# Alisah-Ozcan/GPU-NTT

Measured on AMD Instinct MI355X. Metric: forward-NTTs/sec + achieved HBM GB/s, 64-bit Merge N=2^16 batch=1024, higher is better.
Workload: dtype u64; 1 GPU; Merge-NTT Data64 log2N=16 batch=1024 forward (BASELINE configs[1]); log2N=16, batch_per_gpu=1024, reduction_poly=X_N_minus, modulus=576460756061519873, in_place=True, api=dropin, parallelism=batch-shard x1

## Files before the change

### gpu-ntt_amd/__init__.py

```python
import ctypes
import os
import subprocess
from dataclasses import dataclass
from typing import Optional

import numpy as np

_HERE = os.path.dirname(os.path.abspath(__file__))
LIB_PATH = os.environ.get("GPUNTT_LIB") or os.path.join(_HERE, "lib", "libgpuntt.so")
CSRC = os.path.join(_HERE, "csrc")

FORWARD, INVERSE = 0, 1
PerPolynomial, PerCoefficient = 0, 1
X_N_plus, X_N_minus = 0, 1

GPUNTT_OK = 0
_ERR_INVALID, _ERR_HIP = -1, -2


class GpuNttError(RuntimeError):
    """HipException / CudaException of the C++ API (failed launch)."""


class _M32(ctypes.Structure):
# ... 52 lines not shown
              "innerprod_plan_owns_workspace", "innerprod_plan_destroy", "innerprod_constants",
              "innerprod_reference",
              "keyswitch_plan_workspace_bytes", "keyswitch_plan_scratch_bytes", "keyswitch_plan_create",
              "keyswitch_plan_mod_up", "keyswitch_plan_mod_down", "keyswitch_plan_decompose",
              "keyswitch_plan_switch_digits", "keyswitch_plan_apply", "keyswitch_plan_hoisted_scratch_bytes",
              "keyswitch_plan_rotate_hoisted", "keyswitch_plan_hoisted_sum_scratch_bytes",
              "keyswitch_plan_rotate_hoisted_sum", "keyswitch_plan_multiply_relinearize",
              "keyswitch_plan_multiply_relinearize_sum", "keyswitch_plan_owns_workspace",
              "keyswitch_plan_destroy", "keyswitch_constants", "keyswitch_reference_mod_up",
              "keyswitch_reference_mod_down",
              "keyswitch_plan_workspace_bytes_rescale", "keyswitch_plan_create_rescale",
              "keyswitch_plan_rescale_limbs", "keyswitch_plan_rescale_scratch_bytes",
              "keyswitch_plan_mod_down_rescale", "keyswitch_plan_rescale",
              "keyswitch_plan_multiply_relinearize_rescale", "keyswitch_plan_multiply_relinearize_sum_rescale",
              "keyswitch_plan_rotate_hoisted_sum_rescale", "keyswitch_reference_mod_down_rescale",
              "keyswitch_reference_rescale")
    for s in ("u32", "u64")] + ["gpuntt_release_workspaces", "gpuntt_set_option", "gpuntt_galois_element_u32",
                                "gpuntt_automorphism_index_map"]

ENV_OPTIONS = {"GPUNTT_PATH": ("path", None), "GPUNTT_U32_E32": ("u32_e32", lambda v: int(v, 0)),
               "GPUNTT_TWO_SWEEP_BIG": ("two_sweep_big", None)}


TEST_HOOKS = {"no_scratch", "rns_force_fallback", "u32_e32", "reset_predictions", "two_sweep_big", "baseconv_ksplit",
              "keyswitch_split", "keyswitch_hoist_chunk", "contig_p4"}
TEST_PATHS = {"fast-strict", "generic-capped"}


def set_option(name, value):
    name, value = str(name), str(value)
    if name in TEST_HOOKS or (name == "path" and value in TEST_PATHS):
        return set_test_hook(name, value)
    _check(load_library().gpuntt_set_option(name.encode(), value.encode()))


def set_test_hook(name, value):
    _check(load_library().gpuntt_test_set_hook(str(name).encode(), str(value).encode()))


def contig_p4_launches():
    fn = load_library().gpuntt_test_contig_p4_launches
    fn.restype = ctypes.c_ulonglong
    return int(fn())


def alloc_count():
    fn = load_library().gpuntt_test_alloc_count
    fn.restype = ctypes.c_ulonglong
    return int(fn())


def scratch_stats():
    out = (ctypes.c_ulonglong * 6)()
    _check(load_library().gpuntt_test_scratch_stats(out))
    names = ("graph_owned", "died", "pooled", "reused", "chains_erased", "chains")
    return dict(zip(names, (int(v) for v in out)))


class launch_log:

    def __enter__(self):
        _check(load_library().gpuntt_test_launch_log_start())
        self.kernels = []
        return self

    def __exit__(self, *exc):
# ... 1144 lines not shown
```

### gpu-ntt_amd/csrc/c_api.cpp

```cpp
#include <algorithm>
#include <cstring>
#include <exception>
#include <initializer_list>
#include <stdexcept>
#include <string>
#include <vector>

#include "gpuntt/ntt_4step/ntt_4step.cuh"
#include "gpuntt/ntt_merge/galois.cuh"
#include "gpuntt/ntt_merge/ntt.cuh"
#include "gpuntt/rns/base_conversion.cuh"
#include "gpuntt/rns/inner_product.cuh"
#include "gpuntt/rns/key_switch.cuh"
#include "gpuntt_c.h"
#include "hoisted_rotation_internal.hpp"
#include "test_hooks.h"

namespace gpuntt
{
    namespace host
    {
        template <typename T> void debug_recip_norm(const T* q, T* out, unsigned long long count, hipStream_t stream);
        bool set_test_hook(const char* name, const char* value);
        void launch_log_start();
        size_t launch_log_take(std::string& out, size_t capacity);
        unsigned long long alloc_count();
        void scratch_stats(unsigned long long out[6]);
        unsigned long long contig_p4_launches();
    }
}

using namespace gpuntt;

namespace
{
    thread_local std::string g_last_error;

    template <typename F> int guarded(F&& f)
    {
        try
        {
            f();
            return GPUNTT_OK;
        }
        catch (const std::invalid_argument& e)
        {
            g_last_error = e.what();
            return GPUNTT_ERR_INVALID_ARGUMENT;
        }
        catch (const HipException& e)
        {
            g_last_error = e.what();
            return GPUNTT_ERR_HIP;
        }
        catch (const std::exception& e)
        {
            g_last_error = e.what();
            return GPUNTT_ERR_UNKNOWN;
        }
    }

// ... 420 lines not shown
    }
    int gpuntt_version(void) { return 101; }

    int gpuntt_test_set_hook(const char* name, const char* value)
    {
        return guarded([&] {
            if (!host::set_test_hook(name, value))
                throw std::invalid_argument("Unknown option or value!");
        });
    }
    int gpuntt_test_launch_log_start(void)
    {
        return guarded([] { host::launch_log_start(); });
    }
    int gpuntt_test_launch_log_take(char* buf, int capacity)
    {
        std::string s;
        const size_t room = (buf != nullptr && capacity > 0) ? static_cast<size_t>(capacity - 1) : 0;
        const size_t need = host::launch_log_take(s, room);
        if (buf != nullptr && capacity > 0)
        {
            std::memcpy(buf, s.data(), s.size());
            buf[s.size()] = '\0';
        }
        return static_cast<int>(need) + 1;
    }
    unsigned long long gpuntt_test_alloc_count(void) { return host::alloc_count(); }

    int gpuntt_test_scratch_stats(unsigned long long out[6])
    {
        return guarded([&] { host::scratch_stats(out); });
    }
    unsigned long long gpuntt_test_contig_p4_launches(void) { return host::contig_p4_launches(); }
    int gpuntt_test_keyswitch_hoist_chunk(int word_bytes, int digits, int n_power)
    {
        if ((word_bytes != 4 && word_bytes != 8) || digits < 1 || digits > INNERPROD_MAX_DIGITS || n_power < 1 ||
            n_power > 28)
            return -1;
        return host::hoist_chunk_log(static_cast<size_t>(word_bytes), digits, n_power, host::HOIST_LOG_MAX);
    }
    int gpuntt_test_keyswitch_hoist_sum_chunk(int word_bytes, int digits, int n_power)
    {
        if ((word_bytes != 4 && word_bytes != 8) || digits < 1 || digits > INNERPROD_MAX_DIGITS || n_power < 1 ||
            n_power > 28)
            return -1;
        return host::hoist_chunk_log(static_cast<size_t>(word_bytes), digits, n_power, host::HOIST_SUM_LOG_MAX);
    }

    int gpuntt_galois_element_u32(int steps, int n_power, int conjugation, uint32_t* elt_host)
    {
        GPUNTT_NEED(elt_host)
        return guarded([&] {
            *elt_host = conjugation ? GaloisElementForConjugation(n_power) : GaloisElementForRotation(steps, n_power);
        });
    }
    int gpuntt_automorphism_index_map(int n_power, uint32_t galois_elt, int reduction_poly, int domain,
                                      uint32_t* map_host)
    {
        GPUNTT_NEED(map_host)
        return guarded([&] {
            if (n_power <= 0 || n_power >= 29)
                throw std::invalid_argument("Invalid n_power range!");
            if (reduction_poly != GPUNTT_X_N_PLUS && reduction_poly != GPUNTT_X_N_MINUS)
                throw std::invalid_argument("Invalid reduction_poly!");
            if (domain != GPUNTT_DOMAIN_NTT && domain != GPUNTT_DOMAIN_COEFFICIENT)
                throw std::invalid_argument("Invalid domain!");
// ... 701 lines not shown
```

### gpu-ntt_amd/csrc/contig_p4_map.hpp

```cpp
#pragma once

#if defined(__HIPCC__) || defined(__CUDACC__)
#define GPUNTT_P4_HD __host__ __device__
#else
#define GPUNTT_P4_HD
#endif

namespace gpuntt
{
    namespace kern
    {
        namespace p4
        {
            constexpr int TLOG = 12;
            constexpr int K = 10;
            constexpr int RB = 4;
            constexpr int NT = 256;
            constexpr int POLYS = 1 << (TLOG - K);
            constexpr int ROUNDS = 3;
            constexpr int LDS_ELEMS = (1 << TLOG) + (1 << (TLOG - 4)) + 16 * (POLYS - 1);

            GPUNTT_P4_HD constexpr int window(int r) { return r == 0 ? 6 : (r == 1 ? 4 : 0); }

            GPUNTT_P4_HD constexpr unsigned thread_of(int r, unsigned t)
            {
                return r == 0 ? t : ((t & 15u) | ((t >> 6) << 4) | (((t >> 4) & 3u) << 6));
            }
            GPUNTT_P4_HD constexpr unsigned elem(int r, unsigned t, unsigned j)
            {
                const unsigned u = thread_of(r, t);
                const int w = window(r);
                return (u & ((1u << w) - 1u)) | (j << w) | ((u >> w) << (w + RB));
            }
            GPUNTT_P4_HD constexpr unsigned elem_out(unsigned t, unsigned j)
            {
                return (t & 63u) | ((j & 3u) << 6) | ((t >> 6) << 8) | ((j >> 2) << K);
            }
            GPUNTT_P4_HD constexpr unsigned lds_slot(unsigned e) { return e + (e >> 4) + ((e >> K) << 4); }
            GPUNTT_P4_HD constexpr unsigned long long mem_offset(unsigned e, unsigned long long poly_stride)
            {
                return static_cast<unsigned long long>(e >> K) * poly_stride + (e & ((1u << K) - 1u));
            }
            GPUNTT_P4_HD constexpr unsigned ring_pos(unsigned seg, unsigned e) { return (seg << K) | (e & ((1u << K) - 1u)); }

            GPUNTT_P4_HD constexpr unsigned tw_uniform_index(int n, unsigned seg, unsigned blk, int p, unsigned kk)
            {
                return (1u << (n - 1 - p)) + (((seg << K) | (blk << 8)) >> (p + 1)) + kk;
            }
            GPUNTT_P4_HD constexpr unsigned tw_lane_index(int n, unsigned seg, unsigned t, int p, unsigned kk)
            {
                const unsigned group = ((seg & 3u) << 6) | ((t >> 6) << 4) | (t & 15u);
                return (1u << (n - 1 - p)) + (seg >> 2) * ((8u >> p) * NT) + kk * NT + group;
            }
        }
    }
}
```

### gpu-ntt_amd/csrc/lazy_launch.hpp

```cpp
#pragma once

#include <hip/hip_runtime.h>

#include <string>

#include "launch.hpp"
#include "merge_lazy_kernels.hpp"

namespace gpuntt
{
    namespace host
    {
        constexpr int LAZY_MAX_N_POWER = 28;

        constexpr int lazy_u32_tile_override() { return 0; }
        constexpr int lazy_u64_big_tiles() { return 14; }

        bool lazy_two_sweep_big();
        bool lazy_contig_p4();
        void note_contig_p4_launch();
        unsigned long long contig_p4_launches();
        constexpr int LAZY_P4_N_POWER = 16;
        constexpr unsigned long long lazy_u32_small_batch() { return 0x7fffffffull; }
        template <typename T> inline int lazy_tile_log(int n, bool inverse = false, unsigned long long polys = 0)
        {
            if (sizeof(T) == 8)
            {
                const int big = lazy_u64_big_tiles();
                if (n == 13 && big >= 13)
                    return 13;
                if (n == 14 && big >= 14 && !inverse && polys >= 256)
                    return 14;
                if (n == 21 && big >= 13)
                    return 13;
                if (n == 22 && big >= 14)
                    return 14;
                if ((n == 23 || n == 24) && !inverse && lazy_two_sweep_big())
                    return 14;
                return 12;
            }
            if (n <= 12)
                return 12;
            {
                const unsigned long long small = lazy_u32_small_batch();
                if (n == 13 && small != 0 && (polys == 0 ? small >= 0x7fffffffull : polys <= small))
                    return 13;
            }
            if (n <= 14)
                return 14;
            const int forced = lazy_u32_tile_override();
            if (forced != 0)
                return forced;
            return (n >= 20 && n <= 22) ? 14 : 12;
        }

// ... 504 lines not shown
```

### gpu-ntt_amd/csrc/lazy_launch_impl.hpp

```cpp
#pragma once

#include "lazy_launch.hpp"

namespace gpuntt
{
    namespace host
    {
        template <typename T, int TLOG, bool INV, bool CONTIG, int K, int IN_BOUND, bool LAST, int LIMSEL = 0, bool P4 = false,
                  int CAP = 0>
        inline void launch_lazy_one(const kern::LazyArgsT<T>& a, unsigned grid, hipStream_t stream)
        {
            if constexpr (P4)
                note_contig_p4_launch();
            GPUNTT_LAUNCH_FAMILY(LIMSEL, (kern::merge_pass_lazy<T, TLOG, INV, CONTIG, K, IN_BOUND, LAST, LIMSEL, 0, P4, CAP>), dim3(grid),
                               dim3(kern::LTile<TLOG>::NT), 0, stream, a);
            GPUNTT_HIP_CHECK(hipGetLastError());
        }

        template <typename T, int TLOG, bool INV, int LIMSEL = 0>
        void dispatch_tl(const Pass& p, bool in_first, bool last, const kern::LazyArgsT<T>& a,
                         hipStream_t stream)
        {
            constexpr int LIM = lazy::Mod<T, LIMSEL>::LIMIT;
            constexpr int TILE = kern::LTile<TLOG>::TILE;
            const unsigned long long tiles = (a.total + TILE - 1) >> TLOG;
            if (tiles == 0)
                return;
            if (tiles > 0x7fffffffull)
                throw std::invalid_argument("batch_size * N too large for one launch");
            const unsigned grid = lazy_grid_cap<T, LIMSEL>(tiles, a.go_flag);
            constexpr bool CAPPED = sizeof(T) == 8 && !INV && TLOG == 12 && (LIM == 16 || LIM == 31);
            constexpr int CAP10 = CAPPED ? FwdBounds<CAPPED ? LIM : 16>::CAP10 : LIM;
            if (!CAPPED && p.cap != 0)
                throw std::invalid_argument("internal: no capped hand-off in this kernel family");
#define GPUNTT_ONE(CONTIG_, K_, IN_, LAST_)                                                      \
    return launch_lazy_one<T, TLOG, INV, CONTIG_, K_, IN_, LAST_, LIMSEL>(a, grid, stream)
            if constexpr (sizeof(T) == 8 && TLOG >= 13)
            {
                if (p.contig && p.k == TLOG)
                {
                    if (in_first && last)
                        GPUNTT_ONE(true, TLOG, 1, true);
                    if constexpr (!INV)
                    {
                        if (!in_first && last)
                            GPUNTT_ONE(true, TLOG, LIM, true);
// ... 33 lines not shown
                            case 8: GPUNTT_ONE(true, 8, 1, true);
                            case 9: GPUNTT_ONE(true, 9, 1, true);
                            case 10: GPUNTT_ONE(true, 10, 1, true);
                            case 11: GPUNTT_ONE(true, 11, 1, true);
                            case 12: GPUNTT_ONE(true, 12, 1, true);
                            default: break;
                        }
                    else if constexpr (TLOG == 13)
                    {
                        if (p.k == 13)
                            GPUNTT_ONE(true, 13, 1, true);
                    }
                    else
                        switch (p.k)
                        {
                            case 13: GPUNTT_ONE(true, 13, 1, true);
                            case 14: GPUNTT_ONE(true, 14, 1, true);
                            default: break;
                        }
                }
                else if (!INV && !in_first && last)
                {
                    if constexpr (!INV)
                    {
                        if constexpr (TLOG == 12)
                            switch (p.k)
                            {
                                case 8: GPUNTT_ONE(true, 8, LIM, true);
                                case 9: GPUNTT_ONE(true, 9, LIM, true);
                                case 10:
                                    if constexpr (sizeof(T) == 8)
                                        if (p.p4)
                                        {
                                            if constexpr (CAPPED)
                                                if (fwd_inst_bound(p, TLOG, in_first, last, LIM) == CAP10)
                                                    return launch_lazy_one<T, TLOG, INV, true, 10, CAP10, true, LIMSEL, true>(a, grid, stream);
                                            return launch_lazy_one<T, TLOG, INV, true, 10, LIM, true, LIMSEL, true>(a, grid, stream);
                                        }
                                    if constexpr (CAPPED)
                                        if (fwd_inst_bound(p, TLOG, in_first, last, LIM) == CAP10)
                                            GPUNTT_ONE(true, 10, CAP10, true);
                                    GPUNTT_ONE(true, 10, LIM, true);
                                case 11: GPUNTT_ONE(true, 11, LIM, true);
                                case 12: GPUNTT_ONE(true, 12, LIM, true);
                                default: break;
                            }
                        else if constexpr (TLOG == 14)
                        {
                            if (p.k == 14)
                                GPUNTT_ONE(true, 14, LIM, true);
                            if (p.k == 13)
                                GPUNTT_ONE(true, 13, LIM, true);
                        }
                    }
                }
                else if (INV && in_first && !last)
                {
                    if constexpr (INV)
                    {
                        if constexpr (TLOG == 12)
                            switch (p.k)
                            {
                                case 8: GPUNTT_ONE(true, 8, 1, false);
                                case 9: GPUNTT_ONE(true, 9, 1, false);
                                case 10: GPUNTT_ONE(true, 10, 1, false);
                                case 11: GPUNTT_ONE(true, 11, 1, false);
                                case 12: GPUNTT_ONE(true, 12, 1, false);
                                default: break;
                            }
                        else if constexpr (TLOG == 14)
// ... 371 lines not shown
```

### gpu-ntt_amd/csrc/merge_lazy_kernels.hpp

```cpp
#pragma once

#include "contig_p4_map.hpp"
#include "lazy.hpp"
#include "merge_kernels.hpp"

namespace gpuntt
{
    namespace kern
    {
        template <typename T> struct LazyArgsT
        {
            const void* in;
            T* out;
            const lazy::Tw<T>* tw;
            const Modulus<T>* mods;
            T q;
            T q_bit;
            T q_mu;
            const lazy::Tw<T>* ninv_arr;
            lazy::Tw<T> ninv;
            lazy::NormConst norm;
            const lazy::NormConst* norm_arr;
            const unsigned* go_flag;
            const int* mod_order;
            const int* poly_order;
            const T* mul_in;
            const T* fs_n1;
            const T* fs_n2;
            const T* fs_w;
            int lim;
            int host_allow_31q;
            int n2_log;
            int row_log;
            int batch;
            int col_log;
            int mod_shift;
            unsigned long long total;
            int n;
            int poly_shift;
            int mod_count;
            int p_lo;
            unsigned flags;
        };
        using LazyArgs = LazyArgsT<uint64_t>;

        template <int WL> constexpr int lds_joff(int j)
        {
            return (j << WL) + ((WL >= 4) ? (j << (WL >= 4 ? WL - 4 : 0)) : (j >> (WL < 4 ? 4 - WL : 0)));
        }

        template <int TLOG> struct LTile
        {
            static constexpr int TL = TLOG;
            static constexpr int NT = 1 << (TLOG - R);
            static constexpr int TILE = 1 << TLOG;
            static constexpr int LDS_ELEMS = TILE + (TILE >> 4);
            static constexpr int LDS_ELEMS_FST = TILE + (TILE >> 4) + (TILE >> 5);
        };
        template <int TLOG, bool CONTIG, int K> struct LGeo
        {
            static constexpr int L = CONTIG ? 0 : (TLOG - K);
            static constexpr int NR = (K + R - 1) / R;
        };
        template <int TLOG, bool CONTIG, int K, bool SEG = false> struct LTileMap
        {
            unsigned long long base;
            int p_lo;
            __device__ __forceinline__ explicit LTileMap(unsigned long long flat_base, int row_shift = 0)
                : base(flat_base), p_lo(row_shift)
            {
            }
            __device__ __forceinline__ LTileMap(int n, int pass_p_lo, unsigned long long blk)
            {
                constexpr int L = LGeo<TLOG, CONTIG, K>::L;
                if constexpr (CONTIG)
// ... 123 lines not shown
                                b[j1] = TB;
                            }
                        }
                        g++;
                    }
                    int mx = 0;
                    for (int j = 0; j < EPT; j++)
                    {
                        d.bout[r][j] = b[j];
                        mx = b[j] > mx ? b[j] : mx;
                    }
                    bound_in = mx;
                }
                d.final_bound = (EST && (!whole.ok || whole.out != bound_in)) ? LIMIT + 1 : bound_in;
                return d;
            }
            static constexpr Data d = make();
            static_assert(d.final_bound <= LIMIT, "lazy bound exceeds the headroom");
            static_assert(d.final_bound <= HANDOFF_CAP, "the pass hands over more than its successor was compiled for");
            static_assert(!INV || d.final_bound <= LIMIT / 2, "an inverse pass must hand over values below LIMIT / 2");
        };

        template <typename T, bool INV, bool VQ, bool PLAIN> constexpr bool plans_whole_pass(int limit)
        {
            return !INV && sizeof(T) == 8 && !VQ && PLAIN && (limit == 16 || limit == 31);
        }

        template <int TLOG, typename T = uint32_t> struct LOcc
        {
            static constexpr int WAVES = (TLOG >= 14 && sizeof(T) == 4) ? 8 : 4;
        };

        constexpr int TW_PER_ROUND = EPT - 1;

        template <bool NT_, typename T> __device__ __forceinline__ T ld_stream(const T* p)
        {
            if constexpr (NT_)
                return __builtin_nontemporal_load(p);
            else
                return *p;
        }
        template <bool NT_, typename T> __device__ __forceinline__ void st_stream(T* p, T v)
        {
            if constexpr (NT_)
                __builtin_nontemporal_store(v, p);
            else
                *p = v;
        }

        __device__ __forceinline__ void wave_sync()
        {
            __builtin_amdgcn_fence(__ATOMIC_RELEASE, "wavefront");
            __builtin_amdgcn_wave_barrier();
            __builtin_amdgcn_fence(__ATOMIC_ACQUIRE, "wavefront");
        }

        constexpr int XP_L1 = 5;
        template <int K> __device__ __forceinline__ unsigned xp_swap_fwd(unsigned f)
        {
            constexpr unsigned M = (1u << K) - 1u;
            const unsigned w = f & M;
            return (f & ~M) | ((w & 31u) << (K - XP_L1)) | (w >> XP_L1);
        }
        template <int K> __device__ __forceinline__ unsigned xp_swap_inv(unsigned e)
        {
            return xp_swap_fwd<K>(e);
// ... 24 lines not shown
                else
                    asm volatile("" : "+v"(v[j])::"memory");
            }
        }

        enum class Fst : int
        {
            none = 0,
            nat_rows = 2,
            inv_first = 3
        };
        enum class Xp : int
        {
            none = 0,
            small_fwd = 1,
            small_inv = 2,
            small_nat_fwd = 3,
            small_nat_inv = 4,
            first_gather = 5
        };

        template <typename T, int N> __device__ __forceinline__ void relayout_barrier(T (&loaded)[N])
        {
            pin_loaded(loaded);
            __syncthreads();
        }

        template <typename T, int TLOG, bool INV, bool CONTIG, int K, int IN_BOUND, bool LAST,
                  Fst FST = Fst::none, int LIM = 0, Xp XP = Xp::none, int SKIP = 0, bool VQ = false, int ROWLEN = 0,
                  bool P4 = false, int CAP = 0>
        __device__ __forceinline__ void pass_body(const LazyArgsT<T>& a, T* lds, T q_value, T q_bit, T q_mu,
                                                  int mi, unsigned long long fst_poly = 0,
                                                  unsigned fst_tile = 0, long long blk_override = -1,
                                                  unsigned fst_seg = 0)
        {
            using G = LGeo<TLOG, CONTIG, K>;
            using M = lazy::Mod<T, LIM, VQ>;
            constexpr bool EST = plans_whole_pass<T, INV, VQ, (FST == Fst::none && XP == Xp::none)>(M::LIMIT);
            static_assert(CAP == 0 || EST, "hand-off caps: plain forward 64-bit passes");
            using SCH = PassSched<TLOG, INV, CONTIG, K, IN_BOUND, M::LIMIT, M::TB, SKIP, CAP, EST>;
            using TW = lazy::Tw<T>;
            static_assert(!VQ || (FST == Fst::none && XP == Xp::none && SKIP == 0), "per-lane moduli: plain passes");
            static_assert(!(VQ && CONTIG) || (K >= R && K < TLOG && IN_BOUND == 1 && LAST),
                          "per-lane moduli, contiguous: single-pass transforms of rings of 16 .. tile/2 coefficients");
            static_assert(!P4 || (sizeof(T) == 8 && TLOG == p4::TLOG && !INV && CONTIG && K == p4::K && IN_BOUND != 1 && LAST &&
                                  FST == Fst::none && XP == Xp::none && SKIP == 0 && !VQ),
                          "four-polynomial tile: the forward 64-bit 10-stage last pass");
            constexpr bool HAS_FST = (FST != Fst::none);
            constexpr int TL = TLOG;
            constexpr int NT = LTile<TLOG>::NT;
            constexpr int NR_ = SCH::NR;
            static_assert(!P4 || (SCH::NR == p4::ROUNDS && SCH::wl_of(0) == p4::window(0) && SCH::wl_of(1) == p4::window(1) &&
                                  SCH::wl_of(P4 ? 2 : 0) == p4::window(2) && SCH::stages_of(0) == 2 && SCH::stages_of(1) == 4 &&
                                  SCH::stages_of(P4 ? 2 : 0) == 4 && SCH::first_pos(0) == 9 && SCH::first_pos(1) == 7 &&
                                  SCH::first_pos(P4 ? 2 : 0) == 3),
                          "contig_p4_map.hpp assumes this round schedule");

            constexpr bool MULTI_POLY = CONTIG && (K < TL) && (IN_BOUND == 1) && (LAST || HAS_FST);
            constexpr bool WIO_OK = CONTIG && (!HAS_FST || FST == Fst::inv_first) && !MULTI_POLY && (TL >= 10);
            constexpr int WIO = 6;
            const int t = threadIdx.x;
            constexpr bool SEG = (FST == Fst::nat_rows);
            using Map = LTileMap<TLOG, CONTIG, K, SEG>;
            Map map = P4    ? Map(fst_poly)
                      : SEG ? Map((fst_poly << a.poly_shift) +
                                      ((static_cast<unsigned long long>(fst_tile) << (TL - K)) << a.row_log) +
                                      (static_cast<unsigned long long>(fst_seg) << K),
                                  a.row_log)
                      : HAS_FST ? Map((fst_poly << a.poly_shift) + (static_cast<unsigned long long>(fst_tile) << TL))
                            : Map(a.n, a.p_lo,
                                  blk_override >= 0 ? static_cast<unsigned long long>(blk_override)
                                                    : static_cast<unsigned long long>(blockIdx.x));
            const bool tile_in_range = (CONTIG && !HAS_FST && !P4) ? ((map.base + LTile<TLOG>::TILE) <= a.total) : true;
            if constexpr (!P4)
                if (a.poly_order != nullptr)
                    map.remap_poly(a.poly_order, a.n);
            const unsigned p4_seg = fst_tile;
            const unsigned p4_wave = P4 ? static_cast<unsigned>(__builtin_amdgcn_readfirstlane(t >> 6)) : 0u;
            const unsigned long long p4_stride =
                P4 ? (static_cast<unsigned long long>(a.mods != nullptr ? a.mod_count : 1) << a.n) : 0ull;
            (void) p4_seg;
            (void) p4_wave;
            (void) p4_stride;
            if constexpr (VQ)
            {
                unsigned owner;
                if constexpr (CONTIG)
                    owner = static_cast<unsigned>(map.base >> K) + (static_cast<unsigned>(t) >> (K - R));
                else
                    owner = static_cast<unsigned>(map.flat(elem_of<SCH::wl_of(0)>(t, 0))) & ((1u << a.col_log) - 1u);
                mi = static_cast<int>(owner % static_cast<unsigned>(a.mod_count));
                const Modulus<T> md = a.mods[a.mod_order != nullptr ? a.mod_order[mi] : mi];
                q_value = md.value;
                q_bit = md.bit;
                q_mu = md.mu;
            }
            static_assert(sizeof(T) != 8 || LOcc<TLOG, T>::WAVES <= 4,
                          "64-bit lazy kernels need the 128-VGPR budget (v126 / v127 are named in lazy.hpp)");
            M m;
            m.set(q_value, (a.norm_arr != nullptr) ? a.norm_arr[mi] : a.norm);
            const dev::ModCtx<T> em{q_value, q_bit, q_mu};
            const unsigned long long root_base = static_cast<unsigned long long>(mi) << ((VQ && !CONTIG) ? a.mod_shift : a.n);
            T ninv_w = a.ninv.w, ninv_wp = a.ninv.wp;
            if (LAST && INV && a.ninv_arr != nullptr)
            {
                ninv_w = a.ninv_arr[mi].w;
                ninv_wp = a.ninv_arr[mi].wp;
            }
            const TW ninv{ninv_w, ninv_wp};
            const unsigned nmask = (1u << a.n) - 1u;
            const TW* __restrict__ tw_mod = a.tw + root_base;

            auto load_twiddles = [&](auto r_, TW(&tws)[TW_PER_ROUND]) {
                constexpr int r = decltype(r_)::value;
                constexpr int STAGES = SCH::stages_of(r);
                constexpr int FIRST_POS = SCH::first_pos(r);
                constexpr int WL = SCH::wl_of(r);
                if constexpr (P4)
                {
                    int o4 = 0;
                    static_for<STAGES>([&](auto s_) {
                        constexpr int s = decltype(s_)::value;
                        constexpr int p = FIRST_POS - s;
                        constexpr int CNT = 1 << (R - 1 - (p - WL));
                        const TW* ps = tw_mod + (r == 2 ? p4::tw_lane_index(a.n, p4_seg, static_cast<unsigned>(t), p, 0)
                                                        : p4::tw_uniform_index(a.n, p4_seg, r == 1 ? p4_wave : 0u, p, 0));
                        static_for<CNT>([&](auto k_) {
                            constexpr int kk = decltype(k_)::value;
                            tws[o4 + kk] = ps[r == 2 ? kk * NT : kk];
                        });
                        o4 += CNT;
                    });
                    return;
                }
                constexpr bool UNIFORM = (WL + R == TL) || (WL >= 6);
                const int t_uni = (WL + R == TL) ? 0 : __builtin_amdgcn_readfirstlane(t);
                int off = 0;
                static_for<STAGES>([&](auto s_) {
                    constexpr int s = decltype(s_)::value;
                    constexpr int p = INV ? (FIRST_POS + s) : (FIRST_POS - s);
                    constexpr int jb = p - WL;
                    constexpr int CNT = 1 << (R - 1 - jb);
                    constexpr bool PERM = CONTIG && !MULTI_POLY && !SEG && (WL == 0) && (p <= 2);
                    const int P = map.gpos(p);
                    const unsigned stage_base = 1u << (a.n - 1 - P);
                    const TW* ps;
                    if constexpr (PERM)
                    {
                        const unsigned tile_in_poly = (static_cast<unsigned>(map.flat(0)) & nmask) >> TL;
                        ps = tw_mod + stage_base + tile_in_poly * (CNT * NT) + t;
                    }
                    else
                    {
                        const unsigned idx0 =
                            static_cast<unsigned>(map.flat(elem_of<WL>(UNIFORM ? t_uni : t, 0))) & nmask;
                        ps = tw_mod + stage_base + (idx0 >> (P + 1));
                    }
                    static_for<CNT>([&](auto k_) {
                        constexpr int kk = decltype(k_)::value;
                        if constexpr (CONTIG && !MULTI_POLY && !SEG && (WL != 0) && (p <= 2))
                        {
                            const unsigned e0 = elem_of<WL>(t, kk << (jb + 1));
                            const unsigned tile_in_poly = (static_cast<unsigned>(map.flat(0)) & nmask) >> TL;
                            constexpr int RP = EPT >> (p + 1);
                            tws[off + kk] = tw_mod[stage_base + tile_in_poly * (RP * NT) +
                                                   ((e0 & (EPT - 1)) >> (p + 1)) * NT + (e0 >> R)];
                        }
                        else if constexpr (MULTI_POLY)
                        {
                            constexpr int KOFF = ((kk << (jb + 1 + WL)) & ((1 << K) - 1)) >> (p + 1);
                            tws[off + kk] = ps[KOFF];
                        }
                        else
                        {
                            tws[off + kk] = ps[PERM ? kk * NT : kk];
                        }
                    });
                    off += CNT;
                });
            };

            const bool full_tile = tile_in_range;
            const bool plain_io = full_tile;
            const bool signed_in = (!INV && IN_BOUND == 1 && !HAS_FST) ? ((a.flags & F_SIGNED_IN) != 0u) : false;
            auto to_residue = [&](T x) -> T {
                using S = typename std::make_signed<T>::type;
                return (static_cast<S>(x) < 0) ? static_cast<T>(x + m.q) : x;
            };

            constexpr bool TW_AHEAD = (LOcc<TLOG, T>::WAVES <= 4);

            T v[EPT];
            TW tw_next[TW_PER_ROUND];
            if constexpr (TW_AHEAD)
                load_twiddles(std::integral_constant<int, 0>{}, tw_next);

            static_for<NR_>([&](auto r_) {
                constexpr int r = decltype(r_)::value;
                constexpr int STAGES = SCH::stages_of(r);
                constexpr int FIRST_POS = SCH::first_pos(r);
                constexpr int WL = SCH::wl_of(r);
                constexpr bool DIRECT_IO = (WL >= 4);
                constexpr bool UNIFORM_R = P4 ? (r < 2) : ((WL + R == TL) || (WL >= 6));

                if constexpr (r == 0)
                {
                    auto load_guarded = [&](unsigned long long f) -> T {
                        const bool inside = f < a.total;
                        const T raw = static_cast<const T*>(a.in)[inside ? f : 0ull];
                        T val = raw;
                        if (a.flags & F_SIGNED_IN)
                        {
                            using S = typename std::make_signed<T>::type;
                            val = (static_cast<S>(raw) < 0) ? static_cast<T>(m.q + raw) : raw;
                        }
                        return inside ? val : static_cast<T>(0);
                    };
                    const T* src = static_cast<const T*>(a.in);
                    if constexpr (XP == Xp::small_fwd)
                    {
                        constexpr int XG = 8;
#pragma unroll
                        for (int part = 0; part < EPT / XG; part++)
                        {
                            T tmp[XG];
                            if (plain_io)
                            {
#pragma unroll
                                for (int jj = 0; jj < XG; jj++)
// ... 165 lines not shown
                            {
#pragma unroll
                                for (int j = 0; j < EPT; j++)
                                    tmp[j] = to_residue(tmp[j]);
                            }
                            T* lc = lds + lds_pad(t);
#pragma unroll
                            for (int j = 0; j < EPT; j++)
                                lc[NT * j + ((NT * j) >> 4)] = tmp[j];
                        }
                        else
                        {
#pragma unroll
                            for (int j = 0; j < EPT; j++)
                                lds[lds_pad(t + NT * j)] = load_guarded(map.flat(t + NT * j));
                        }
                        __syncthreads();
                        const T* lw = lds + lds_pad(elem_of<WL>(t, 0));
#pragma unroll
                        for (int j = 0; j < EPT; j++)
                            v[j] = lw[lds_joff<WL>(j)];
                    }
                }
                else
                {
                    const T* lw = lds + (P4 ? static_cast<int>(p4::lds_slot(p4::elem(r, static_cast<unsigned>(t), 0)))
                                            : lds_pad(elem_of<WL>(t, 0)));
#pragma unroll
                    for (int j = 0; j < EPT; j++)
                        v[j] = lw[lds_joff<WL>(j)];
                }

                TW tw_cur[TW_PER_ROUND];
                if constexpr (TW_AHEAD)
                {
#pragma unroll
                    for (int i = 0; i < TW_PER_ROUND; i++)
                        tw_cur[i] = tw_next[i];
                }
                else
                {
                    load_twiddles(r_, tw_cur);
                }

                int off = 0;
                static_for<STAGES>([&](auto s_) {
                    constexpr int s = decltype(s_)::value;
                    constexpr int p = INV ? (FIRST_POS + s) : (FIRST_POS - s);
                    constexpr int jb = p - WL;
                    if constexpr (!INV && SCH::d.ku[r][s][0] == lazy::CT_EST)
                    {
                        if (m.hi_norm())
                            static_for<EPT / 2>([&](auto h_) {
                                constexpr int h = decltype(h_)::value;
                                constexpr int j0 = (h & ((1 << jb) - 1)) | ((h >> jb) << (jb + 1));
                                v[j0] = m.template reduce_2q<true>(v[j0]);
                            });
                        else
                            static_for<EPT / 2>([&](auto h_) {
                                constexpr int h = decltype(h_)::value;
                                constexpr int j0 = (h & ((1 << jb) - 1)) | ((h >> jb) << (jb + 1));
                                v[j0] = m.template reduce_2q<false>(v[j0]);
                            });
                    }
                    static_for<EPT / 2>([&](auto h_) {
                        constexpr int h = decltype(h_)::value;
                        constexpr int j0 = (h & ((1 << jb) - 1)) | ((h >> jb) << (jb + 1));
// ... 261 lines not shown
                        }
                        else
                        {
#pragma unroll
                            for (int j = 0; j < EPT; j++)
                            {
                                const unsigned long long f = map.flat(t + NT * j);
                                if (f < a.total)
                                {
                                    const T x = lds[lds_pad(t + NT * j)];
                                    a.out[f] = (PMUL_OK && mul_in != nullptr) ? em.mul(x, mul_in[f]) : x;
                                }
                            }
                        }
                    }
                }
                else
                {
                    if constexpr (TW_AHEAD)
                        load_twiddles(std::integral_constant<int, r + 1>{}, tw_next);
                    T* lw = lds + (P4 ? static_cast<int>(p4::lds_slot(p4::elem(r, static_cast<unsigned>(t), 0)))
                                      : lds_pad(elem_of<WL>(t, 0)));
#pragma unroll
                    for (int j = 0; j < EPT; j++)
                        lw[lds_joff<WL>(j)] = v[j];
                    if constexpr (P4 && r == 0)
                        relayout_barrier(v);
                    else if constexpr (WL <= 6 && SCH::wl_of(r + 1 < NR_ ? r + 1 : r) <= 6)
                        wave_sync();
                    else
                        __syncthreads();
                }
            });
        }

        constexpr unsigned GO_GENERIC = 0u, GO_LAZY = 1u, GO_LAZY_8Q = 2u, GO_LAZY_4Q = 3u, GO_LAZY_31Q = 4u;
        __host__ __device__ constexpr int family_rank(unsigned state)
        {
            return state == GO_LAZY_31Q ? 0 : (state == GO_LAZY ? 1 : (state == GO_LAZY_8Q ? 2 : (state == GO_LAZY_4Q ? 3 : -1)));
        }
        template <typename T> struct SlowArgs
        {
            const void* in;
            T* out;
            const T* mul_in;
            const int* poly_order;
            unsigned long long polys;
            int col_log;
            unsigned flags;
            int inverse;
            int enabled;
            int force;
        };

        template <typename T, int LIM> __device__ __forceinline__ bool not_my_call(const unsigned* go_flag, unsigned flags = 0u)
        {
            constexpr unsigned mine = sizeof(T) != 8 ? GO_LAZY
                                      : (LIM == 4 ? GO_LAZY_4Q : (LIM == 8 ? GO_LAZY_8Q : (LIM == 31 ? GO_LAZY_31Q : GO_LAZY)));
            if (go_flag == nullptr)
                return false;
            const unsigned st = *go_flag;
            return (flags & F_VETO_ONLY) ? (st == GO_GENERIC) : (st != mine);
        }

        template <typename T, int LIM> struct WalksTiles
        {
// ... 121 lines not shown
            for (int e = t; e < N; e += NT)
                out[e] = INV ? m.mul(lds[e], ninv) : lds[e];
        }

        template <typename T, int TLOG, bool INV, bool CONTIG, int K, int IN_BOUND, bool LAST, int LIM = 0, int SKIP = 0,
                  bool P4 = false, int CAP = 0>
        __global__ __launch_bounds__(LTile<TLOG>::NT, (LOcc<TLOG, T>::WAVES)) void merge_pass_lazy(LazyArgsT<T> a)
        {
            using M = lazy::Mod<T, LIM>;
            constexpr int SK = INV ? SKIP : 0;
            using SCH = PassSched<TLOG, INV, CONTIG, K, IN_BOUND, M::LIMIT, M::TB, SK>;
            constexpr bool NEEDS_LDS = (SCH::NR > 1) || (SCH::wl_of(0) < 4);
            __shared__ T lds[P4 ? p4::LDS_ELEMS : (NEEDS_LDS ? LTile<TLOG>::LDS_ELEMS : 1)];

            if constexpr (SKIP != 0 && TLOG == 12 && CONTIG)
                if (self_fallback_call<T, LIM>(a))
                {
                    if constexpr (INV)
                        fs_phase2_chunk<T, true, LTile<12>::NT>(a, blockIdx.x, a.n, fs_modulus(a), fs_ninv(a));
                    else
                        fs_phase2_chunk<T, false, LTile<12>::NT>(a, blockIdx.x, a.n - a.n2_log, fs_modulus(a), T(0));
                    return;
                }
            if (not_my_call<T, LIM>(a.go_flag, a.flags))
                return;
            for_each_block<WalksTiles<T, LIM>::value>(
                static_cast<unsigned>((a.total + LTile<TLOG>::TILE - 1) >> TLOG), [&](unsigned bidx, unsigned nblk) {
            T qv = a.q, qb = a.q_bit, qm = a.q_mu;
            int mi = 0;
            const unsigned bx = (a.flags & F_REVERSE) ? (nblk - 1u - bidx) : bidx;
            if constexpr (P4)
            {
                const unsigned mc = (a.mods != nullptr) ? static_cast<unsigned>(a.mod_count) : 1u;
                const int seg_log = a.n - K;
                const unsigned seg = uniform32(bx & ((1u << seg_log) - 1u));
                const unsigned pm = bx >> seg_log;
                mi = static_cast<int>(uniform32(pm % mc));
                const unsigned long long poly0 = static_cast<unsigned long long>(pm / mc) * (4u * mc) + static_cast<unsigned>(mi);
                if (a.mods != nullptr)
                {
                    const Modulus<T> md = a.mods[mi];
                    qv = md.value;
                    qb = md.bit;
                    qm = md.mu;
                }
                pass_body<T, TLOG, INV, CONTIG, K, IN_BOUND, LAST, Fst::none, LIM, Xp::none, SK, false, 0, true, CAP>(
                    a, lds, qv, qb, qm, mi, uniform64((poly0 << a.n) + (static_cast<unsigned long long>(seg) << K)), seg);
                return;
            }
            long long blk = static_cast<long long>(bx);
            if (a.batch > 1)
            {
                unsigned poly, tile;
                poly_minor_order(bx, static_cast<unsigned>(a.batch), a.n - TLOG, poly, tile, a.flags);
                blk = static_cast<long long>(
                    uniform64((static_cast<unsigned long long>(poly) << (a.n - TLOG)) | tile));
            }
            if (a.mods != nullptr)
            {
                const LTileMap<TLOG, CONTIG, K> map(a.n, a.p_lo, static_cast<unsigned long long>(blk));
                unsigned long long poly = map.flat(0) >> a.poly_shift;
                if constexpr (CONTIG && K < TLOG && K - R >= 6 && IN_BOUND == 1 && LAST)
                    poly += threadIdx.x >> (K - R);
                mi = static_cast<int>(uniform32(static_cast<unsigned>(poly % static_cast<unsigned>(a.mod_count))));
                const Modulus<T> md = a.mods[a.mod_order != nullptr ? a.mod_order[mi] : mi];
                qv = md.value;
                qb = md.bit;
                qm = md.mu;
            }
            pass_body<T, TLOG, INV, CONTIG, K, IN_BOUND, LAST, Fst::none, LIM, Xp::none, SK, false, 0, false, CAP>(a, lds, qv, qb,
                                                                                                                   qm, mi, 0, 0, blk);
                });
        }

        template <typename T> struct VqLim
        {
            static constexpr int LIM = (sizeof(T) == 8) ? 4 : 0;
        };
        template <typename T, bool INV, int K, int IN_BOUND, bool LAST>
        __global__ __launch_bounds__(LTile<12>::NT, (LOcc<12, T>::WAVES)) void merge_pass_lazy_vq(LazyArgsT<T> a)
// ... 174 lines not shown
```

### gpu-ntt_amd/csrc/prep.hip

```cpp
#include <atomic>
#include <cctype>
#include <cstdlib>
#include <initializer_list>
#include <string>
#include <map>
#include <tuple>
#include <mutex>
#include <stdexcept>
#include <thread>
#include <vector>

#include "lazy_launch.hpp"
#include "rns_predict.hpp"

namespace gpuntt
{
    namespace kern
    {
        template <typename T> __device__ __forceinline__ T shoup_quotient(T w, T q)
        {
            T rem = w, quo = 0;
#pragma unroll 8
            for (int i = 0; i < static_cast<int>(8 * sizeof(T)); i++)
            {
// ... 479 lines not shown
            const unsigned k = (n > 1) ? (__brev(i) >> (33 - n)) : 0u;
            const unsigned n2 = 1u << log_n2;
            const unsigned j = k & (n2 - 1u), m = k >> log_n2;
            const unsigned long long widx =
                inverse ? (static_cast<unsigned long long>(n2) + (__brev(j) >> (32 - log_n2)))
                        : ((static_cast<unsigned long long>(n2) << (log_n1 - 1)) + j);
            T w = w_table[widx];
            if (m != 0u)
                w = mulmod_r<T>(w, n1_table[__brev(m) >> (33 - log_n1)], q, rinv);
            if (fold && slot == 1)
                w = mulmod_r<T>(w, ninv, q, rinv);
            ws[slot] = lazy::Tw<T>{w, shoup_quotient_r<T>(w, q, rinv)};
        }

    }

    namespace host
    {
        void baseconv_set_ksplit(int v);
        void keyswitch_set_split(int v);
        void keyswitch_set_hoist_chunk(int v);
        namespace
        {
            struct OptionValues
            {
                int path = 0;
                int no_scratch = 0;
                int check_4step = 1;
                int rns_predict = 1;
                int rns_force_fallback = 0;
                int u32_e32 = 0x1f000;
                int two_sweep_big = 0;
                int contig_p4 = 1;
            };
            std::mutex g_opt_mutex;
            std::atomic<int> g_reset_predictions{0};
            OptionValues g_opt;
            std::atomic<unsigned> g_opt_generation{1};
            thread_local OptionValues t_opt;
            thread_local unsigned t_opt_generation = 0;
            thread_local int t_scope_depth = 0;

            void refresh_snapshot()
            {
                const unsigned gen = g_opt_generation.load(std::memory_order_acquire);
                if (gen != t_opt_generation)
                {
                    std::lock_guard<std::mutex> lock(g_opt_mutex);
                    t_opt = g_opt;
                    t_opt_generation = g_opt_generation.load(std::memory_order_relaxed);
                }
            }
            const OptionValues& options()
            {
                if (t_scope_depth == 0)
                    refresh_snapshot();
                return t_opt;
            }

            bool set_option_impl(const char* name, const char* value, bool test_hooks)
            {
                if (name == nullptr || value == nullptr)
                    return false;
                const std::string k(name), v(value);
                const bool hex = value[0] == '0' && (value[1] == 'x' || value[1] == 'X');
                const char* digits = hex ? value + 2 : value;
                char* end = nullptr;
                const long lv = std::strtol(digits, &end, hex ? 16 : 10);
                const bool is_num = (hex ? std::isxdigit(static_cast<unsigned char>(digits[0]))
                                         : std::isdigit(static_cast<unsigned char>(digits[0]))) != 0 && *end == '\0';
                const int iv = static_cast<int>(lv);
                const bool bit = is_num && (lv == 0 || lv == 1);
                std::lock_guard<std::mutex> lock(g_opt_mutex);
                if (k == "path")
                {
                    const int m = v == "generic" ? 1 : v == "fast" ? 2 : (v == "default" || v.empty()) ? 0
                                  : (test_hooks && v == "fast-strict") ? 3 : (test_hooks && v == "generic-capped") ? 4 : -1;
                    if (m < 0)
                        return false;
                    g_opt.path = m;
                }
                else if (k == "check_4step_tables" && bit)
                    g_opt.check_4step = iv;
                else if (k == "rns_predict" && bit)
                    g_opt.rns_predict = iv;
                else if (test_hooks && k == "no_scratch" && bit)
                    g_opt.no_scratch = iv;
                else if (test_hooks && k == "rns_force_fallback" && bit)
                    g_opt.rns_force_fallback = iv;
                else if (test_hooks && k == "u32_e32" && is_num && lv >= 0 && (lv & ~0x1f000L) == 0)
                    g_opt.u32_e32 = iv;
                else if (test_hooks && k == "two_sweep_big" && bit)
                    g_opt.two_sweep_big = iv;
                else if (test_hooks && k == "contig_p4" && bit)
                    g_opt.contig_p4 = iv;
                else if (test_hooks && k == "baseconv_ksplit" && is_num && lv >= 0 && lv <= 16)
                    baseconv_set_ksplit(iv);
                else if (test_hooks && k == "keyswitch_split" && is_num && lv >= 0 && lv <= 64)
                    keyswitch_set_split(iv);
                else if (test_hooks && k == "keyswitch_hoist_chunk" && is_num && (lv == 0 || (lv >= 6 && lv <= 13)))
                    keyswitch_set_hoist_chunk(iv);
                else if (test_hooks && k == "reset_predictions" && is_num && lv == 1)
                    g_reset_predictions.store(1, std::memory_order_relaxed);
                else
                    return false;
                g_opt_generation.fetch_add(1, std::memory_order_release);
                return true;
            }
        }

        bool set_option(const char* name, const char* value) { return set_option_impl(name, value, false); }
        bool set_test_hook(const char* name, const char* value) { return set_option_impl(name, value, true); }
        unsigned lazy_e32_mask() { return static_cast<unsigned>(options().u32_e32); }
        int forced_path() { return options().path; }
        bool lazy_two_sweep_big() { return options().two_sweep_big != 0; }
        bool lazy_contig_p4() { return options().contig_p4 != 0; }
        static bool rns_predict_enabled() { return options().rns_predict != 0; }
        static bool rns_force_fallback() { return options().rns_force_fallback != 0; }
        bool check_4step_tables() { return options().check_4step != 0; }

        namespace
        {
            std::atomic<int> g_log_on{0};
            std::mutex g_log_mutex;
            std::vector<std::string> g_log;
        }
        void note_launch(const char* kernel_expr, int family)
        {
            if (g_log_on.load(std::memory_order_relaxed) == 0)
                return;
            std::string k(kernel_expr);
            const size_t a = k.find("kern::");
            if (a != std::string::npos)
                k = k.substr(a + 6);
            const size_t b = k.find_first_of("<)( ,");
            if (b != std::string::npos)
                k = k.substr(0, b);
            if (family >= 0)
                k += ":" + std::to_string(family);
            std::lock_guard<std::mutex> lock(g_log_mutex);
            g_log.push_back(k);
        }
        namespace
        {
            std::atomic<unsigned long long> g_contig_p4_launches{0};
        }
        void note_contig_p4_launch() { g_contig_p4_launches.fetch_add(1, std::memory_order_relaxed); }
        unsigned long long contig_p4_launches() { return g_contig_p4_launches.load(std::memory_order_relaxed); }
        void launch_log_start()
        {
            std::lock_guard<std::mutex> lock(g_log_mutex);
            g_log.clear();
            g_log_on.store(1, std::memory_order_relaxed);
        }
        size_t launch_log_take(std::string& out, size_t capacity)
        {
            std::lock_guard<std::mutex> lock(g_log_mutex);
            g_log_on.store(0, std::memory_order_relaxed);
            size_t need = 0;
            for (const std::string& e : g_log)
                need += e.size() + 1;
            need -= need != 0 ? 1 : 0;
            out.clear();
            if (need > capacity)
                return need;
            out.reserve(need);
            for (const std::string& e : g_log)
                out += (out.empty() ? "" : " ") + e;
            g_log.clear();
            return need;
        }

        namespace
        {
            std::atomic<unsigned long long> g_alloc_calls{0};
            inline void note_alloc_call() { g_alloc_calls.fetch_add(1, std::memory_order_relaxed); }
        }
        unsigned long long alloc_count() { return g_alloc_calls.load(std::memory_order_relaxed); }

        namespace
// ... 508 lines not shown
```

Baseline: 2.631 million NTT/s.

## Let contig-p4 blocks loop over multiple poly groups with resident twiddles

```diff
diff --git a/gpu-ntt_amd/__init__.py b/gpu-ntt_amd/__init__.py
--- a/gpu-ntt_amd/__init__.py
+++ b/gpu-ntt_amd/__init__.py
@@ -108,6 +108,12 @@
     if name in TEST_HOOKS or (name == "path" and value in TEST_PATHS):
         return set_test_hook(name, value)
     _check(load_library().gpuntt_set_option(name.encode(), value.encode()))
+
+
+def contig_p4_last_grid():
+    fn = load_library().gpuntt_test_contig_p4_last_grid
+    fn.restype = ctypes.c_uint
+    return int(fn())
 
 
 def set_test_hook(name, value):
diff --git a/gpu-ntt_amd/csrc/c_api.cpp b/gpu-ntt_amd/csrc/c_api.cpp
--- a/gpu-ntt_amd/csrc/c_api.cpp
+++ b/gpu-ntt_amd/csrc/c_api.cpp
@@ -27,6 +27,7 @@
         unsigned long long alloc_count();
         void scratch_stats(unsigned long long out[6]);
         unsigned long long contig_p4_launches();
+        unsigned contig_p4_last_grid();
     }
 }
 
@@ -513,6 +514,7 @@
         return guarded([&] { host::scratch_stats(out); });
     }
     unsigned long long gpuntt_test_contig_p4_launches(void) { return host::contig_p4_launches(); }
+    unsigned gpuntt_test_contig_p4_last_grid(void) { return host::contig_p4_last_grid(); }
     int gpuntt_test_keyswitch_hoist_chunk(int word_bytes, int digits, int n_power)
     {
         if ((word_bytes != 4 && word_bytes != 8) || digits < 1 || digits > INNERPROD_MAX_DIGITS || n_power < 1 ||
diff --git a/gpu-ntt_amd/csrc/contig_p4_map.hpp b/gpu-ntt_amd/csrc/contig_p4_map.hpp
--- a/gpu-ntt_amd/csrc/contig_p4_map.hpp
+++ b/gpu-ntt_amd/csrc/contig_p4_map.hpp
@@ -52,6 +52,43 @@
                 const unsigned group = ((seg & 3u) << 6) | ((t >> 6) << 4) | (t & 15u);
                 return (1u << (n - 1 - p)) + (seg >> 2) * ((8u >> p) * NT) + kk * NT + group;
             }
+
+            struct BlockGroups
+            {
+                unsigned seg;
+                unsigned modulus;
+                unsigned chunk;
+                unsigned first;
+                unsigned last;
+            };
+            GPUNTT_P4_HD constexpr unsigned chunk_count(unsigned groups, unsigned per_block)
+            {
+                return (groups + per_block - 1u) / per_block;
+            }
+            GPUNTT_P4_HD constexpr unsigned long long grid_blocks(int n, unsigned mod_count, unsigned groups, unsigned per_block)
+            {
+                return (static_cast<unsigned long long>(mod_count) << (n - K)) * chunk_count(groups, per_block);
+            }
+            GPUNTT_P4_HD constexpr BlockGroups block_groups(int n, unsigned mod_count, unsigned groups, unsigned per_block,
+                                                            unsigned bx)
+            {
+                const unsigned cm = bx >> (n - K);
+                const unsigned chunk = cm / mod_count;
+                const unsigned first = chunk * per_block;
+                const unsigned left = groups - first;
+                return BlockGroups{bx & ((1u << (n - K)) - 1u), cm % mod_count, chunk, first,
+                                   first + (left < per_block ? left : per_block)};
+            }
+            GPUNTT_P4_HD constexpr unsigned long long tile_base(int n, unsigned mod_count, unsigned group, unsigned modulus,
+                                                                unsigned seg)
+            {
+                return ((static_cast<unsigned long long>(group) * (POLYS * mod_count) + modulus) << n) +
+                       (static_cast<unsigned long long>(seg) << K);
+            }
+            GPUNTT_P4_HD constexpr unsigned long long group_step(int n, unsigned mod_count)
+            {
+                return static_cast<unsigned long long>(POLYS * mod_count) << n;
+            }
         }
     }
 }
diff --git a/gpu-ntt_amd/csrc/lazy_launch.hpp b/gpu-ntt_amd/csrc/lazy_launch.hpp
--- a/gpu-ntt_amd/csrc/lazy_launch.hpp
+++ b/gpu-ntt_amd/csrc/lazy_launch.hpp
@@ -18,9 +18,25 @@
 
         bool lazy_two_sweep_big();
         bool lazy_contig_p4();
-        void note_contig_p4_launch();
+        void note_contig_p4_launch(unsigned grid);
+        unsigned contig_p4_last_grid();
         unsigned long long contig_p4_launches();
         constexpr int LAZY_P4_N_POWER = 16;
+        int lazy_contig_p4_groups();
+        constexpr unsigned p4_groups_per_block(unsigned , unsigned ) { return 1; }
+        template <typename T> inline unsigned p4_launch_shape(kern::LazyArgsT<T>& a)
+        {
+            const unsigned mc = a.mods != nullptr ? static_cast<unsigned>(a.mod_count) : 1u;
+            const unsigned long long groups = (a.total >> a.n) / (4ull * mc);
+            const unsigned long long blocks1 = kern::p4::grid_blocks(a.n, mc, 1, 1) * groups;
+            if (groups == 0 || blocks1 > 0x7fffffffull)
+                throw std::invalid_argument("batch_size * N too large for one launch");
+            const int hook = lazy_contig_p4_groups();
+            a.p4_groups = static_cast<unsigned>(groups);
+            a.p4_per_block = hook != 0 ? static_cast<unsigned>(hook)
+                                       : p4_groups_per_block(a.p4_groups, mc);
+            return static_cast<unsigned>(kern::p4::grid_blocks(a.n, mc, a.p4_groups, a.p4_per_block));
+        }
         constexpr unsigned long long lazy_u32_small_batch() { return 0x7fffffffull; }
         template <typename T> inline int lazy_tile_log(int n, bool inverse = false, unsigned long long polys = 0)
         {
diff --git a/gpu-ntt_amd/csrc/lazy_launch_impl.hpp b/gpu-ntt_amd/csrc/lazy_launch_impl.hpp
--- a/gpu-ntt_amd/csrc/lazy_launch_impl.hpp
+++ b/gpu-ntt_amd/csrc/lazy_launch_impl.hpp
@@ -11,7 +11,7 @@
         inline void launch_lazy_one(const kern::LazyArgsT<T>& a, unsigned grid, hipStream_t stream)
         {
             if constexpr (P4)
-                note_contig_p4_launch();
+                note_contig_p4_launch(grid);
             GPUNTT_LAUNCH_FAMILY(LIMSEL, (kern::merge_pass_lazy<T, TLOG, INV, CONTIG, K, IN_BOUND, LAST, LIMSEL, 0, P4, CAP>), dim3(grid),
                                dim3(kern::LTile<TLOG>::NT), 0, stream, a);
             GPUNTT_HIP_CHECK(hipGetLastError());
@@ -111,10 +111,12 @@
                                     if constexpr (sizeof(T) == 8)
                                         if (p.p4)
                                         {
+                                            kern::LazyArgsT<T> a4 = a;
+                                            const unsigned grid4 = p4_launch_shape(a4);
                                             if constexpr (CAPPED)
                                                 if (fwd_inst_bound(p, TLOG, in_first, last, LIM) == CAP10)
-                                                    return launch_lazy_one<T, TLOG, INV, true, 10, CAP10, true, LIMSEL, true>(a, grid, stream);
-                                            return launch_lazy_one<T, TLOG, INV, true, 10, LIM, true, LIMSEL, true>(a, grid, stream);
+                                                    return launch_lazy_one<T, TLOG, INV, true, 10, CAP10, true, LIMSEL, true>(a4, grid4, stream);
+                                            return launch_lazy_one<T, TLOG, INV, true, 10, LIM, true, LIMSEL, true>(a4, grid4, stream);
                                         }
                                     if constexpr (CAPPED)
                                         if (fwd_inst_bound(p, TLOG, in_first, last, LIM) == CAP10)
diff --git a/gpu-ntt_amd/csrc/merge_lazy_kernels.hpp b/gpu-ntt_amd/csrc/merge_lazy_kernels.hpp
--- a/gpu-ntt_amd/csrc/merge_lazy_kernels.hpp
+++ b/gpu-ntt_amd/csrc/merge_lazy_kernels.hpp
@@ -41,6 +41,8 @@
             int mod_count;
             int p_lo;
             unsigned flags;
+            unsigned p4_groups;
+            unsigned p4_per_block;
         };
         using LazyArgs = LazyArgsT<uint64_t>;
 
@@ -230,6 +232,7 @@
         };
 
         constexpr int TW_PER_ROUND = EPT - 1;
+        constexpr int P4_TW_RES_FROM = 7;
 
         template <bool NT_, typename T> __device__ __forceinline__ T ld_stream(const T* p)
         {
@@ -320,7 +323,7 @@
         __device__ __forceinline__ void pass_body(const LazyArgsT<T>& a, T* lds, T q_value, T q_bit, T q_mu,
                                                   int mi, unsigned long long fst_poly = 0,
                                                   unsigned fst_tile = 0, long long blk_override = -1,
-                                                  unsigned fst_seg = 0)
+                                                  unsigned fst_seg = 0, unsigned p4_iters = 1)
         {
             using G = LGeo<TLOG, CONTIG, K>;
             using M = lazy::Mod<T, LIM, VQ>;
@@ -370,6 +373,7 @@
             (void) p4_seg;
             (void) p4_wave;
             (void) p4_stride;
+            (void) p4_iters;
             if constexpr (VQ)
             {
                 unsigned owner;
@@ -399,7 +403,9 @@
             const unsigned nmask = (1u << a.n) - 1u;
             const TW* __restrict__ tw_mod = a.tw + root_base;
 
-            auto load_twiddles = [&](auto r_, TW(&tws)[TW_PER_ROUND]) {
+            unsigned p4_seg_it = p4_seg;
+            (void) p4_seg_it;
+            auto load_twiddles = [&](auto r_, TW(&tws)[TW_PER_ROUND], bool resident = false) {
                 constexpr int r = decltype(r_)::value;
                 constexpr int STAGES = SCH::stages_of(r);
                 constexpr int FIRST_POS = SCH::first_pos(r);
@@ -411,12 +417,25 @@
                         constexpr int s = decltype(s_)::value;
                         constexpr int p = FIRST_POS - s;
                         constexpr int CNT = 1 << (R - 1 - (p - WL));
-                        const TW* ps = tw_mod + (r == 2 ? p4::tw_lane_index(a.n, p4_seg, static_cast<unsigned>(t), p, 0)
-                                                        : p4::tw_uniform_index(a.n, p4_seg, r == 1 ? p4_wave : 0u, p, 0));
-                        static_for<CNT>([&](auto k_) {
-                            constexpr int kk = decltype(k_)::value;
-                            tws[o4 + kk] = ps[r == 2 ? kk * NT : kk];
-                        });
+                        if constexpr (r == 2)
+                        {
+                            const TW* ps = tw_mod + p4::tw_lane_index(a.n, p4_seg, static_cast<unsigned>(t), p, 0);
+                            static_for<CNT>([&](auto k_) {
+                                constexpr int kk = decltype(k_)::value;
+                                if (resident == (o4 + kk >= P4_TW_RES_FROM))
+                                    tws[o4 + kk] = ps[kk * NT];
+                            });
+                        }
+                        else
+                        {
+                            using TWC = const __attribute__((address_space(4))) TW;
+                            TWC* ps = (TWC*) (tw_mod + p4::tw_uniform_index(a.n, p4_seg_it, r == 1 ? p4_wave : 0u, p, 0));
+                            static_for<CNT>([&](auto k_) {
+                                constexpr int kk = decltype(k_)::value;
+                                tws[o4 + kk].w = ps[kk].w;
+                                tws[o4 + kk].wp = ps[kk].wp;
+                            });
+                        }
                         o4 += CNT;
                     });
                     return;
@@ -480,9 +499,18 @@
 
             T v[EPT];
             TW tw_next[TW_PER_ROUND];
-            if constexpr (TW_AHEAD)
+            TW tw_res[TW_PER_ROUND];
+            if constexpr (P4)
+                load_twiddles(std::integral_constant<int, NR_ - 1>{}, tw_res, true);
+            else if constexpr (TW_AHEAD)
                 load_twiddles(std::integral_constant<int, 0>{}, tw_next);
 
+            auto rounds = [&]() {
+            if constexpr (P4)
+            {
+                asm volatile("" : "+s"(p4_seg_it));
+                load_twiddles(std::integral_constant<int, 0>{}, tw_next);
+            }
             static_for<NR_>([&](auto r_) {
                 constexpr int r = decltype(r_)::value;
                 constexpr int STAGES = SCH::stages_of(r);
@@ -714,7 +742,17 @@
                 }
 
                 TW tw_cur[TW_PER_ROUND];
-                if constexpr (TW_AHEAD)
+                if constexpr (P4 && r == NR_ - 1)
+                {
+#pragma unroll
+                    for (int i = 0; i < TW_PER_ROUND; i++)
+                    {
+                        if (i >= P4_TW_RES_FROM)
+                            asm volatile("" : "+v"(tw_res[i].w), "+v"(tw_res[i].wp));
+                        tw_cur[i] = i >= P4_TW_RES_FROM ? tw_res[i] : tw_next[i];
+                    }
+                }
+                else if constexpr (TW_AHEAD)
                 {
 #pragma unroll
                     for (int i = 0; i < TW_PER_ROUND; i++)
@@ -1042,6 +1080,20 @@
                         __syncthreads();
                 }
             });
+            };
+            if constexpr (P4)
+            {
+                for (unsigned it = 0;;)
+                {
+                    rounds();
+                    if (++it >= p4_iters)
+                        break;
+                    map.base += p4::group_step(a.n, a.mods != nullptr ? static_cast<unsigned>(a.mod_count) : 1u);
+                    relayout_barrier(v);
+                }
+            }
+            else
+                rounds();
         }
 
         constexpr unsigned GO_GENERIC = 0u, GO_LAZY = 1u, GO_LAZY_8Q = 2u, GO_LAZY_4Q = 3u, GO_LAZY_31Q = 4u;
@@ -1229,11 +1281,9 @@
             if constexpr (P4)
             {
                 const unsigned mc = (a.mods != nullptr) ? static_cast<unsigned>(a.mod_count) : 1u;
-                const int seg_log = a.n - K;
-                const unsigned seg = uniform32(bx & ((1u << seg_log) - 1u));
-                const unsigned pm = bx >> seg_log;
-                mi = static_cast<int>(uniform32(pm % mc));
-                const unsigned long long poly0 = static_cast<unsigned long long>(pm / mc) * (4u * mc) + static_cast<unsigned>(mi);
+                const p4::BlockGroups bg = p4::block_groups(a.n, mc, a.p4_groups, a.p4_per_block, bx);
+                const unsigned seg = uniform32(bg.seg);
+                mi = static_cast<int>(uniform32(bg.modulus));
                 if (a.mods != nullptr)
                 {
                     const Modulus<T> md = a.mods[mi];
@@ -1242,7 +1292,8 @@
                     qm = md.mu;
                 }
                 pass_body<T, TLOG, INV, CONTIG, K, IN_BOUND, LAST, Fst::none, LIM, Xp::none, SK, false, 0, true, CAP>(
-                    a, lds, qv, qb, qm, mi, uniform64((poly0 << a.n) + (static_cast<unsigned long long>(seg) << K)), seg);
+                    a, lds, qv, qb, qm, mi, uniform64(p4::tile_base(a.n, mc, bg.first, bg.modulus, bg.seg)), seg, -1, 0,
+                    uniform32(bg.last - bg.first));
                 return;
             }
             long long blk = static_cast<long long>(bx);
diff --git a/gpu-ntt_amd/csrc/prep.hip b/gpu-ntt_amd/csrc/prep.hip
--- a/gpu-ntt_amd/csrc/prep.hip
+++ b/gpu-ntt_amd/csrc/prep.hip
@@ -535,6 +535,7 @@
                 int u32_e32 = 0x1f000;
                 int two_sweep_big = 0;
                 int contig_p4 = 1;
+                int contig_p4_groups = 0;
             };
             std::mutex g_opt_mutex;
             std::atomic<int> g_reset_predictions{0};
@@ -597,6 +598,8 @@
                     g_opt.two_sweep_big = iv;
                 else if (test_hooks && k == "contig_p4" && bit)
                     g_opt.contig_p4 = iv;
+                else if (test_hooks && k == "contig_p4_groups" && is_num && (lv == 0 || lv == 1 || lv == 2 || lv == 4 || lv == 8 || lv == 16))
+                    g_opt.contig_p4_groups = iv;
                 else if (test_hooks && k == "baseconv_ksplit" && is_num && lv >= 0 && lv <= 16)
                     baseconv_set_ksplit(iv);
                 else if (test_hooks && k == "keyswitch_split" && is_num && lv >= 0 && lv <= 64)
@@ -618,6 +621,7 @@
         int forced_path() { return options().path; }
         bool lazy_two_sweep_big() { return options().two_sweep_big != 0; }
         bool lazy_contig_p4() { return options().contig_p4 != 0; }
+        int lazy_contig_p4_groups() { return options().contig_p4_groups; }
         static bool rns_predict_enabled() { return options().rns_predict != 0; }
         static bool rns_force_fallback() { return options().rns_force_fallback != 0; }
         bool check_4step_tables() { return options().check_4step != 0; }
@@ -647,8 +651,14 @@
         namespace
         {
             std::atomic<unsigned long long> g_contig_p4_launches{0};
-        }
-        void note_contig_p4_launch() { g_contig_p4_launches.fetch_add(1, std::memory_order_relaxed); }
+            std::atomic<unsigned> g_contig_p4_last_grid{0};
+        }
+        void note_contig_p4_launch(unsigned grid)
+        {
+            g_contig_p4_last_grid.store(grid, std::memory_order_relaxed);
+            g_contig_p4_launches.fetch_add(1, std::memory_order_relaxed);
+        }
+        unsigned contig_p4_last_grid() { return g_contig_p4_last_grid.load(std::memory_order_relaxed); }
         unsigned long long contig_p4_launches() { return g_contig_p4_launches.load(std::memory_order_relaxed); }
         void launch_log_start()
         {
```

Result: no change. 2.655 million NTT/s, median of 6 (+0.9%).
